# Ellon/pgslam

Hardware: AMD Instinct MI355X
Metric: ICP-converged scans/sec at 100k-pt scan vs 1M-pt local map (higher is better)
Workload: dtype f32; 1 GPU; scan-to-map ICP, 100000-pt Velodyne-shaped scan vs 1000000-pt local map, <=30 iterations (BASELINE.json configs[1]); distinct_scans=64, matcher=grid, streams=1, parallelism=1 independent replica(s), one process per GPU

## Files before the change

pgslam_amd/csrc/k_minimise.inc:

```

__device__ __forceinline__ void accumulate_pair(double *acc, double w, double px, double py, double pz, double qx,
                                                double qy, double qz, double nx, double ny, double nz)
{
    const double dx = px - qx, dy = py - qy, dz = pz - qz;
    const double e = (nx * dx + ny * dy) + nz * dz;
    double J[6];
    J[0] = py * nz - pz * ny;
    J[1] = pz * nx - px * nz;
    J[2] = px * ny - py * nx;
    J[3] = nx; J[4] = ny; J[5] = nz;
    int k = 0;
#pragma unroll
    for (int a = 0; a < 6; a++)
#pragma unroll
        for (int b = a; b < 6; b++) acc[k++] += w * (J[a] * J[b]);
#pragma unroll
    for (int a = 0; a < 6; a++) acc[21 + a] -= w * (J[a] * e);
    acc[27] += w;
    acc[28] += 1.0;
    acc[29] += w * (e * e);
}

template <int NT>
__device__ __forceinline__ void block_reduce_store(double *acc, double *__restrict__ out)
{
    __shared__ double red[kReduceBlock / 64][NT];
    const int lane = threadIdx.x & 63, wid = threadIdx.x >> 6;
#pragma unroll
    for (int k = 0; k < NT; k++) {
        const double v = wave_sum(acc[k]);
        if (lane == 0) red[wid][k] = v;
    }
    __syncthreads();
    if (threadIdx.x < NT) {
        double s = 0.0;
#pragma unroll
        for (int w = 0; w < kReduceBlock / 64; w++) s += red[w][threadIdx.x];
        out[threadIdx.x] = s;
    }
}

template <typename T>
__device__ __forceinline__ void accumulate_pair_p2p(double *acc, double w, T px, T py, T pz, T qx, T qy, T qz)
{
    const double p[3] = {(double)px, (double)py, (double)pz}, q[3] = {(double)qx, (double)qy, (double)qz};
#pragma unroll
    for (int a = 0; a < 3; a++) { acc[a] += w * p[a]; acc[3 + a] += w * q[a]; }
#pragma unroll
    for (int a = 0; a < 3; a++)
#pragma unroll
        for (int b = 0; b < 3; b++) acc[6 + 3 * a + b] += w * (q[a] * p[b]);
    const double dx = (double)(T)(px - qx), dy = (double)(T)(py - qy), dz = (double)(T)(pz - qz);
    acc[27] += w;
    acc[28] += 1.0;
    acc[29] += sqrt((dx * dx + dy * dy) + dz * dz);
}

template <typename T>
__device__ __forceinline__ void normalized3(T &x, T &y, T &z)
{
    const T zz = (x * x + y * y) + z * z;
    if (zz > (T)0) { const T s = sqrt(zz); x = x / s; y = y / s; z = z / s; }
}

template <typename T>
__device__ __forceinline__ T robust_weight(const RobustDev<T> &rb, T dd, T s2)
{
    const T e2 = dd / s2;
    T w = (T)0;
    switch (rb.fct) {
    case 1: w = (T)1 / ((T)1 + e2 / rb.k2); break;
    case 2: w = exp(-(e2 / rb.k2)); break;
    case 3: { const T t = rb.k + e2; w = e2 >= rb.k ? ((T)4 * rb.k2) / (t * t) : (T)1; break; }
    case 4: { const T t = rb.k + e2; w = rb.k2 / (t * t); break; }
    case 5: { const T t = (T)1 - e2 / rb.k2; w = e2 >= rb.k2 ? (T)0 : t * t; break; }
    case 6: w = e2 >= rb.k2 ? rb.k / sqrt_rn_t(e2) : (T)1; break;
    default: w = (T)1 / sqrt_rn_t(e2); break;
    }
    if (sizeof(T) == 8 && w <= (T)1e-50) w = (T)1e-50;
    if (rb.cut && e2 >= rb.a2) w = (T)0;
    return w;
}

template <typename T>
__device__ __forceinline__ T gd_weight(int mode, T thr, T v, T gmax)
{
    if (mode == PGICP_DESC_FILTER_LARGER) return v > thr ? (T)1 : (T)0;
    if (mode == PGICP_DESC_FILTER_SMALLER) return v < thr ? (T)1 : (T)0;
    return gmax > (T)0 ? v / gmax : (T)0;
}

template <typename T, typename S>
__device__ __forceinline__ T pair_filter_weight(const S *Tc, bool use_nrm, const T *qn, T bx, T by, T bz, T normal_cos, bool robust,
                                                const RobustDev<T> &rb, T dd, T rs2, bool gd, int gd_mode, T gd_thr, T gv, T gmax)
{
    if (use_nrm) {
        T ax = ((T)Tc[0] * qn[0] + (T)Tc[1] * qn[1]) + (T)Tc[2] * qn[2];
        T ay = ((T)Tc[4] * qn[0] + (T)Tc[5] * qn[1]) + (T)Tc[6] * qn[2];
        T az = ((T)Tc[8] * qn[0] + (T)Tc[9] * qn[1]) + (T)Tc[10] * qn[2];
        normalized3<T>(ax, ay, az);
        normalized3<T>(bx, by, bz);
        if (((ax * bx + ay * by) + az * bz) < normal_cos) return (T)0;
    }
    T w = (T)1;
    if (robust) w = robust_weight<T>(rb, dd, rs2);
    if (gd) w = w * gd_weight<T>(gd_mode, gd_thr, gv, gmax);
    return w;
}

template <typename T, int MIN, bool GEN>
__global__ __launch_bounds__(kReduceBlock) void k_p2plane_reduce(const ProblemDev *__restrict__ probs,
                                                                  const MapDev<T> *__restrict__ maps,
                                                                  const T *__restrict__ rd_pre, const T *__restrict__ rd_nrm,
                                                                  const int *__restrict__ slot,
                                                                  const T *__restrict__ d2, double *__restrict__ partials,
                                                                  int max_blocks, const int *__restrict__ active, T normal_cos, RobustDev<T> rb,
                                                                  const int *__restrict__ scan_pos, int gd_mode, T gd_thr)
{
    const int prob = active[blockIdx.y];
    const ProblemDev &P = probs[prob];
    if (P.done) return;
    const int tile = xcd_tile(blockIdx.x, gridDim.x);
    const bool robust = GEN && rb.fct != 0;
    const T rs2 = (T)P.robust_s2;
    const int knn = GEN ? P.knn : 1;
    const int np = GEN ? pairs_n(P) : P.n;
    const long long poff = GEN ? pairs_off(P) : P.off;
    if (tile * kReduceSpan >= np) return;
    const MapDev<T> M = maps[P.map];
    const T limit = (T)P.limit;
    const bool use_nrm = GEN && rd_nrm != nullptr;
    const bool need_nrm = MIN == 0 || use_nrm;
    const bool gd = GEN && gd_mode != PGICP_DESC_FILTER_OFF;
    const T gmax = GEN ? Bits<T>::val((typename Bits<T>::U)P.gd_key) : (T)0;
    double acc[kSys];
#pragma unroll
    for (int k = 0; k < kSys; k++) acc[k] = 0.0;
    using V4 = typename Vec4<T>::type;
    for (int rnd = 0; rnd < kReduceRounds; ++rnd) {
    const int base = tile * kReduceSpan + rnd * (kReduceBlock * kReduceItems);
    if (base >= np) break;
    int ss[kReduceItems];
    bool keep[kReduceItems];
    T dds[GEN ? kReduceItems : 1];
    int es[kReduceItems];
#pragma unroll
    for (int it = 0; it < kReduceItems; it++) {
        const int pos = base + it * kReduceBlock + threadIdx.x;
        int e = pos;
        if (scan_pos && pos < np) e = knn == 1 ? scan_pos[P.off + pos] : scan_pos[P.off + pos / knn] * knn + pos % knn;
        es[it] = e;
        ss[it] = -1;
        T dd = Bits<T>::inf();
        if (pos < np) { dd = d2[poff + e]; ss[it] = slot[poff + e]; }
        keep[it] = ss[it] >= 0 && dd <= limit;
        if constexpr (GEN) dds[it] = dd;
    }
    V4 mp[kReduceItems], mn[kReduceItems];
    T qv[kReduceItems][3], qn[kReduceItems][3];
    T gv[GEN ? kReduceItems : 1];
#pragma unroll
    for (int it = 0; it < kReduceItems; it++) {
        const int e = es[it];
        const int s = keep[it] ? ss[it] : 0;
        const int i = keep[it] ? (knn == 1 ? e : e / knn) : 0;
        if (need_nrm) { mp[it] = M.nrm[2 * (long long)s]; mn[it] = M.nrm[2 * (long long)s + 1]; }
        else mp[it] = M.pts[s];
        const T *q = rd_pre + 3 * (P.off + i);
        qv[it][0] = q[0]; qv[it][1] = q[1]; qv[it][2] = q[2];
        if constexpr (GEN) {
            if (use_nrm) { const T *n = rd_nrm + 3 * (P.off + i); qn[it][0] = n[0]; qn[it][1] = n[1]; qn[it][2] = n[2]; }
            if (gd) gv[it] = M.val[s - (keep[it] ? M.first : 0)];
        }
    }
#pragma unroll
    for (int it = 0; it < kReduceItems; it++) {
        if (keep[it]) {
            double wgt = 1.0;
            if constexpr (GEN) {
                const T w = pair_filter_weight<T>(tcur_of<T>(P), use_nrm, qn[it], use_nrm ? mn[it].x : (T)0, use_nrm ? mn[it].y : (T)0,
                                                  use_nrm ? mn[it].z : (T)0, normal_cos, robust, rb, dds[it], rs2, gd, gd_mode, gd_thr,
                                                  gd ? gv[it] : (T)0, gmax);
                if (w == (T)0) continue;
                wgt = (double)w;
            }
            T px, py, pz;
            apply_T<T>(tcur_of<T>(P), qv[it][0], qv[it][1], qv[it][2], px, py, pz);
            if (MIN == 0)
                accumulate_pair(acc, wgt, (double)px, (double)py, (double)pz, (double)mp[it].x, (double)mp[it].y, (double)mp[it].z,
                                (double)mn[it].x, (double)mn[it].y, (double)mn[it].z);
            else
                accumulate_pair_p2p<T>(acc, wgt, px, py, pz, mp[it].x, mp[it].y, mp[it].z);
        }
    }
    }
    block_reduce_store<kSys>(acc, partials + ((long long)prob * max_blocks + tile) * kSys);
}

template <typename T, int MIN>
__global__ __launch_bounds__(kReduceBlock) void k_error_stats(const MapDev<T> *__restrict__ maps, int map,
                                                               const int *__restrict__ slot_of, const T *__restrict__ rd,
                                                               int stride, const int *__restrict__ ids,
                                                               const T *__restrict__ w, int n, int knn, T mx, T my, T mz,
                                                               double *__restrict__ partials)
{
    const MapDev<T> M = maps[map];
    double acc[kSys];
#pragma unroll
    for (int k = 0; k < kSys; k++) acc[k] = 0.0;
    for (int it = 0; it < kReduceItems * kReduceRounds; it++) {
        const int e = blockIdx.x * kReduceSpan + it * kReduceBlock + threadIdx.x;
        if (e < n * knn) {
            const int i = knn == 1 ? e : e / knn;
            const T wi = w[e];
            const int id = ids[e];
            if (id >= 0 && wi != (T)0) {
                const T px = rd[(long long)i * stride] - mx, py = rd[(long long)i * stride + 1] - my,
                        pz = rd[(long long)i * stride + 2] - mz;
                const int s = slot_of[id];
                const auto mp = M.pts[s];
                if (MIN == 0) {
                    const auto mn = M.nrm[2 * (long long)s + 1];
                    accumulate_pair(acc, (double)wi, (double)px, (double)py, (double)pz, (double)mp.x, (double)mp.y,
                                    (double)mp.z, (double)mn.x, (double)mn.y, (double)mn.z);
                } else
                    accumulate_pair_p2p<T>(acc, (double)wi, px, py, pz, mp.x, mp.y, mp.z);
            }
        }
    }
    block_reduce_store<kSys>(acc, partials + (long long)blockIdx.x * kSys);
}

__device__ __forceinline__ double sum_partials_256(const double *__restrict__ part, int nb, int nt, double (*lds)[32])
{
    const int v = threadIdx.x & 31, grp = threadIdx.x >> 5;
    double s = 0.0;
    if (v < nt)
        for (int b = grp; b < nb; b += 8) s += part[(long long)b * nt + v];
    lds[grp][v] = s;
    __syncthreads();
    double tot = 0.0;
    if (threadIdx.x < 32) {
#pragma unroll
        for (int k = 0; k < 8; k++) tot += lds[k][threadIdx.x];
    }
    return tot;
}

__global__ __launch_bounds__(256) void k_sum_partials(const double *__restrict__ partials, int max_blocks, int nt,
                                                       const ProblemDev *__restrict__ probs ,
                                                       int nb_uniform, double *__restrict__ out)
{
    const int p = blockIdx.x;
    int nb = nb_uniform;
    if (probs) {
        nb = (pairs_n(probs[p]) + kReduceSpan - 1) / kReduceSpan;
        if (probs[p].status != PGICP_ST_OK) nb = 0;
    }
    __shared__ double red[8][32];
    const double *src = partials + (long long)p * max_blocks * nt;
    for (int v0 = 0; v0 < nt; v0 += 32) {
        const int v = threadIdx.x & 31, grp = threadIdx.x >> 5;
        double s = 0.0;
        if (v0 + v < nt)
            for (int b = grp; b < nb; b += 8) s += src[(long long)b * nt + v0 + v];
        __syncthreads();
        red[grp][v] = s;
        __syncthreads();
        if (threadIdx.x < 32 && v0 + threadIdx.x < nt) {
            double tot = 0.0;
#pragma unroll
            for (int k = 0; k < 8; k++) tot += red[k][threadIdx.x];
            out[(long long)p * nt + v0 + threadIdx.x] = tot;
        }
    }
}

__device__ __forceinline__ void single_bookkeeping(int *single_host_flag, int *__restrict__ single_stamp,
                                                   int *__restrict__ single_queue_counters, int done)
{
    if (!single_stamp) return;
    const int stamp = *single_stamp + 1;
    *single_stamp = stamp;
    if (single_queue_counters)
        for (int t = 0; t < 4; ++t) { single_queue_counters[8 + t] = single_queue_counters[t]; single_queue_counters[t] = 0; }
    if (single_host_flag) {
        __hip_atomic_store(single_host_flag, done, __ATOMIC_RELAXED, __HIP_MEMORY_SCOPE_SYSTEM);
        __hip_atomic_store(single_host_flag + 1, stamp, __ATOMIC_RELEASE, __HIP_MEMORY_SCOPE_SYSTEM);
    }
}

template <typename T>
__global__ __launch_bounds__(256) void k_solve_update(ProblemDev *__restrict__ probs, const double *__restrict__ partials,
                                                       int max_blocks, ChainDev<T> ch, int *__restrict__ n_done,
                                                       const int *__restrict__ active, int *single_host_flag,
                                                       int *__restrict__ single_stamp, int *__restrict__ single_queue_counters)
{
    const int prob = active[blockIdx.x];
    ProblemDev &P = probs[prob];
    if (P.done) {
        if (threadIdx.x == 0) single_bookkeeping(single_host_flag, single_stamp, single_queue_counters, 1);
        return;
    }
    __shared__ double sys[kSys];
    __shared__ double red[8][32];
    const int nb = (pairs_n(P) + kReduceSpan - 1) / kReduceSpan;
    const double tot = sum_partials_256(partials + (long long)prob * max_blocks * kSys, nb, kSys, red);
    if (threadIdx.x < kSys) {
        sys[threadIdx.x] = tot;
        P.sys[threadIdx.x] = tot;
    }
    __syncthreads();
    if (threadIdx.x != 0) return;
    P.gd_last = P.gd_key;
    P.gd_key = 0;
    int status = PGICP_ST_OK;
    if (P.n_finite == 0 || !(sys[28] > 0.0)) status = PGICP_ST_NO_MATCH;
    if (status == PGICP_ST_OK) {
        double x[6], dT[16], Tn[16];
        if (ch.minimizer == 1) P.rank = solve_p2point(sys, dT);
        else if (ch.force4dof) {
            double s4[27];
            for (int i = 0; i < 27; i++) s4[i] = sys[i];
            constrain_4dof(s4);
            P.rank = solve6(s4, ch.rank_rel_tol, x) - 2;
            delta_T(x, dT);
        }
        else {
            P.rank = solve6(sys, ch.rank_rel_tol, x);
            delta_T(x, dT);
        }
        for (int i = 0; i < 16; i++) { P.T_prev[i] = P.T_iter[i]; P.dT[i] = dT[i]; }
        mat4_mul(dT, P.T_iter, Tn);
        for (int i = 0; i < 16; i++) P.T_iter[i] = Tn[i];
        for (int i = 0; i < 12; i++) { P.Tcur_prev[i] = P.Tcur[i]; P.Tcur[i] = Tn[i]; P.Tcur_prev_f[i] = P.Tcur_f[i]; P.Tcur_f[i] = (float)Tn[i]; }
        P.n_kept = (int)sys[28];
        P.iters += 1;
        const int f = checker_check(P.chk, Tn, ch.max_iters, ch.min_rot, ch.min_trans, ch.smooth, ch.bound_rot, ch.bound_trans);
        if (f & 8) status = PGICP_ST_NAN;
        else if (f & 16) status = PGICP_ST_BOUND;
        else {
            if (f & 2) P.converged = 1;
            if (f & 4) P.max_iter_reached = 1;
            if (!(f & 1)) { P.done = 1; atomicAdd(n_done, 1); }
        }
    }
    if (status != PGICP_ST_OK) {
        P.status = status;
        P.done = 1;
        atomicAdd(n_done, 1);
    }
    single_bookkeeping(single_host_flag, single_stamp, single_queue_counters, P.done ? 1 : 0);
}

__global__ __launch_bounds__(1024) void k_compact_active(const ProblemDev *__restrict__ probs, int P, int *__restrict__ active,
                                                         int *host_flag, int *__restrict__ stamp_counter, int *__restrict__ queue_counters)
{
    int stamp = 0;
    if (threadIdx.x == 0) { stamp = *stamp_counter + 1; *stamp_counter = stamp; }
    if (queue_counters && threadIdx.x < 4) { queue_counters[8 + threadIdx.x] = queue_counters[threadIdx.x]; queue_counters[threadIdx.x] = 0; }
    __shared__ int lds[32];
    __shared__ int base_live, base_done;
    if (threadIdx.x == 0) { base_live = 0; base_done = 0; }
    __syncthreads();
    int live_cnt = 0;
    for (int p = threadIdx.x; p < P; p += 1024) live_cnt += probs[p].done ? 0 : 1;
    int tot;
    block_exclusive_scan_1024(live_cnt, lds, tot);
    const int n_live = tot;
    for (int b = 0; b < P; b += 1024) {
        const int p = b + threadIdx.x;
        const int is_live = (p < P && !probs[p].done) ? 1 : 0;
        const int is_done = (p < P && probs[p].done) ? 1 : 0;
        int tl, td;
        const int el = block_exclusive_scan_1024(is_live, lds, tl);
        const int ed = block_exclusive_scan_1024(is_done, lds, td);
        if (is_live) active[base_live + el] = p;
        if (is_done) active[n_live + base_done + ed] = p;
        __syncthreads();
        if (threadIdx.x == 0) { base_live += tl; base_done += td; }
        __syncthreads();
    }
    if (host_flag && threadIdx.x == 0) {
        __hip_atomic_store(host_flag, P - n_live, __ATOMIC_RELAXED, __HIP_MEMORY_SCOPE_SYSTEM);
        __hip_atomic_store(host_flag + 1, stamp, __ATOMIC_RELEASE, __HIP_MEMORY_SCOPE_SYSTEM);
    }
}

__global__ __launch_bounds__(256) void k_reopen(ProblemDev *__restrict__ probs, int P)
{
    const int p = blockIdx.x * blockDim.x + threadIdx.x;
    if (p < P && probs[p].status == PGICP_ST_OK) probs[p].done = 0;
}
void launch_reopen(hipStream_t st, ProblemDev *probs, int P)
{
    hipLaunchKernelGGL(k_reopen, dim3((P + 255) / 256), dim3(256), 0, st, probs, P);
}

int knn_trace_set(int sorted_index)
{
#ifdef PGICP_KNN_STATS
    return hipMemcpyToSymbol(HIP_SYMBOL(g_trace_i), &sorted_index, sizeof(int)) == hipSuccess ? 0 : -1;
#else
    (void)sorted_index;
    return -1;
#endif
}

int knn_phase_read(unsigned long long out[48], int reset)
{
#ifdef PGICP_PHASE_STATS
    static unsigned long long h[64 * 48];
    if (hipMemcpyFromSymbol(h, HIP_SYMBOL(g_phase), sizeof h) != hipSuccess) return -1;
    for (int k = 0; k < 48; k++) {
        out[k] = 0;
        const bool is_max = k == 32 + 12 || k == 32 + 13;
        for (int c = 0; c < 64; c++) out[k] = is_max ? std::max(out[k], h[c * 48 + k]) : out[k] + h[c * 48 + k];
    }
    if (reset) { std::memset(h, 0, sizeof h); (void)hipMemcpyToSymbol(HIP_SYMBOL(g_phase), h, sizeof h); }
    {
        unsigned long long b[16];
        if (hipMemcpyFromSymbol(b, HIP_SYMBOL(g_ball), sizeof b) == hipSuccess && b[0])
            std::fprintf(stderr, "      ball walk: %llu waves; per wave: %.1f open lanes, %.1f trips, %.1f items in %.2f evaluations; %.1f rows per open lane\n",
                         b[0], (double)b[1] / b[0], (double)b[2] / b[0], (double)b[4] / b[0], (double)b[5] / b[0], b[1] ? (double)b[7] / b[1] : 0.0);
        if (reset) { std::memset(b, 0, sizeof b); (void)hipMemcpyToSymbol(HIP_SYMBOL(g_ball), b, sizeof b); }
    }
    {
        unsigned long long w[16];
        if (hipMemcpyFromSymbol(w, HIP_SYMBOL(g_slow_worst), sizeof w) == hipSuccess && w[0])
            std::fprintf(stderr, "      slowest entry: %llu cycles [fetch %llu seed %llu look-ups %llu points %llu walk %llu finish %llu]; square of %llu rows, %llu with points, %llu long, %llu candidates; bounded %llu capped %llu, result at %llu mm\n",
                         w[0], w[1], w[2], w[3], w[4], w[5], w[6], w[8], w[9], w[10], w[11], w[12], w[13], w[14]);
        if (reset) { std::memset(w, 0, sizeof w); (void)hipMemcpyToSymbol(HIP_SYMBOL(g_slow_worst), w, sizeof w); }
    }
    return 0;
#else
    (void)out; (void)reset;
    return -1;
#endif
}

int knn_stats_read(unsigned long long out[56], int reset)
{
#ifdef PGICP_KNN_STATS
    if (hipMemcpyFromSymbol(out, HIP_SYMBOL(g_knn_stats), 56 * sizeof(unsigned long long)) != hipSuccess) return -1;
    if (reset) { unsigned long long z[56] = {0}; (void)hipMemcpyToSymbol(HIP_SYMBOL(g_knn_stats), z, sizeof z); }
    return 0;
#else
    (void)out; (void)reset;
    return -1;
#endif
}

int knn_dump_setup(long long total, int passes)
{
#ifdef PGICP_KNN_STATS
    unsigned *c = nullptr; float *d = nullptr;
    if (hipMalloc((void **)&c, sizeof(unsigned) * total * passes) != hipSuccess || hipMalloc((void **)&d, sizeof(float) * total * passes) != hipSuccess) return -1;
    (void)hipMemset(c, 0, sizeof(unsigned) * total * passes);
    (void)hipMemset(d, 0, sizeof(float) * total * passes);
    (void)hipMemcpyToSymbol(HIP_SYMBOL(g_cnt_dump), &c, sizeof c);
    (void)hipMemcpyToSymbol(HIP_SYMBOL(g_d2_dump), &d, sizeof d);
    (void)hipMemcpyToSymbol(HIP_SYMBOL(g_dump_total), &total, sizeof total);
    (void)hipMemcpyToSymbol(HIP_SYMBOL(g_dump_passes), &passes, sizeof passes);
    return 0;
#else
    (void)total; (void)passes;
    return -1;
#endif
}
int knn_dump_read(unsigned *cnt, float *d2, long long n)
{
#ifdef PGICP_KNN_STATS
    unsigned *c = nullptr; float *d = nullptr;
    (void)hipDeviceSynchronize();
    (void)hipMemcpyFromSymbol(&c, HIP_SYMBOL(g_cnt_dump), sizeof c);
    (void)hipMemcpyFromSymbol(&d, HIP_SYMBOL(g_d2_dump), sizeof d);
    if (!c || !d) return -1;
    if (hipMemcpy(cnt, c, sizeof(unsigned) * n, hipMemcpyDeviceToHost) != hipSuccess || hipMemcpy(d2, d, sizeof(float) * n, hipMemcpyDeviceToHost) != hipSuccess) return -1;
    return 0;
#else
    (void)cnt; (void)d2; (void)n;
    return -1;
#endif
}

void launch_compact_active(hipStream_t st, const ProblemDev *probs, int P, int *active, int *host_flag, int *stamp_counter,
                           int *queue_counters)
{
    hipLaunchKernelGGL(k_compact_active, dim3(1), dim3(1024), 0, st, probs, P, active, host_flag, stamp_counter, queue_counters);
}

template <typename T, bool GD>
__global__ __launch_bounds__(kReduceBlock) void k_cov_reduce(const ProblemDev *__restrict__ probs,
                                                              const MapDev<T> *__restrict__ maps,
                                                              const T *__restrict__ rd_pre, const T *__restrict__ rd_nrm,
                                                              const int *__restrict__ slot,
                                                              const T *__restrict__ d2, double *__restrict__ partials,
                                                              int max_blocks, T normal_cos, RobustDev<T> rb, const int *__restrict__ scan_pos,
                                                              int gd_mode, T gd_thr)
{
    const ProblemDev &P = probs[blockIdx.y];
    if (P.status != PGICP_ST_OK) return;
    const int np = pairs_n(P), knn = P.knn;
    const long long poff = pairs_off(P);
    if (blockIdx.x * kReduceSpan >= np) return;
    const MapDev<T> M = maps[P.map];
    const T limit = (T)P.limit;
    double alpha, beta, gamma;
    small_angles(P.dT, alpha, beta, gamma);
    const double t_x = P.dT[3], t_y = P.dT[7], t_z = P.dT[11];
    double Tp[12];
#pragma unroll
    for (int k = 0; k < 12; k++) Tp[k] = P.T_prev[k];
    double acc[kCovTerms];
#pragma unroll
    for (int k = 0; k < kCovTerms; k++) acc[k] = 0.0;
    for (int it = 0; it < kReduceItems * kReduceRounds; it++) {
        const int pos = blockIdx.x * kReduceSpan + it * kReduceBlock + threadIdx.x;
        if (pos >= np) continue;
        const int e = !scan_pos ? pos : knn == 1 ? scan_pos[P.off + pos] : scan_pos[P.off + pos / knn] * knn + pos % knn;
        const T dd = d2[poff + e];
        const int s = slot[poff + e];
        if (s < 0 || !(dd <= limit)) continue;
        if constexpr (GD) {
            T w = rb.fct != 0 ? robust_weight<T>(rb, dd, (T)P.robust_s2) : (T)1;
            w = w * gd_weight<T>(gd_mode, gd_thr, M.val[s - M.first], Bits<T>::val((typename Bits<T>::U)P.gd_last));
            if (w == (T)0) continue;
        } else {
            if (rb.fct != 0 && robust_weight<T>(rb, dd, (T)P.robust_s2) == (T)0) continue;
        }
        const int i = knn == 1 ? e : e / knn;
        const T *q = rd_pre + 3 * (P.off + i);
        T pxt, pyt, pzt;
        apply_T<T>(Tp, q[0], q[1], q[2], pxt, pyt, pzt);
        const auto mp = M.nrm[2 * (long long)s];
        const auto mn = M.nrm[2 * (long long)s + 1];
        if (rd_nrm) {
            const T *n = rd_nrm + 3 * (P.off + i);
            T ax = ((T)Tp[0] * n[0] + (T)Tp[1] * n[1]) + (T)Tp[2] * n[2];
            T ay = ((T)Tp[4] * n[0] + (T)Tp[5] * n[1]) + (T)Tp[6] * n[2];
            T az = ((T)Tp[8] * n[0] + (T)Tp[9] * n[1]) + (T)Tp[10] * n[2];
            T bx = mn.x, by = mn.y, bz = mn.z;
            normalized3<T>(ax, ay, az);
            normalized3<T>(bx, by, bz);
            if (((ax * bx + ay * by) + az * bz) < normal_cos) continue;
        }
        const double px = pxt, py = pyt, pz = pzt, qx = mp.x, qy = mp.y, qz = mp.z, nx = mn.x, ny = mn.y, nz = mn.z;
        const double rr = sqrt((px * px + py * py) + pz * pz);
        const double rdx = px / rr, rdy = py / rr, rdz = pz / rr;
        const double qr = sqrt((qx * qx + qy * qy) + qz * qz);
        const double qdx = qx / qr, qdy = qy / qr, qdz = qz / qr;
        const double n_alpha = nz * rdy - ny * rdz;
        const double n_beta = nx * rdz - nz * rdx;
        const double n_gamma = ny * rdx - nx * rdy;
        double E = nx * (px - gamma * py + beta * pz + t_x - qx);
        E += ny * (gamma * px + py - alpha * pz + t_y - qy);
        E += nz * (-beta * px + alpha * py + pz + t_z - qz);
        double Nr = nx * (rdx - gamma * rdy + beta * rdz);
        Nr += ny * (gamma * rdx + rdy - alpha * rdz);
        Nr += nz * (-beta * rdx + alpha * rdy + rdz);
        const double Nq = -((nx * qdx + ny * qdy) + nz * qdz);
        const double er = E + rr * Nr;
        const double h[6] = {nx, ny, nz, rr * n_alpha, rr * n_beta, rr * n_gamma};
        const double gr[6] = {nx * Nr, ny * Nr, nz * Nr, n_alpha * er, n_beta * er, n_gamma * er};
        const double gq[6] = {nx * Nq, ny * Nq, nz * Nq, qr * n_alpha * Nq, qr * n_beta * Nq, qr * n_gamma * Nq};
        int k = 0;
#pragma unroll
        for (int a = 0; a < 6; a++)
#pragma unroll
            for (int b = a; b < 6; b++) {
                acc[k] += h[a] * h[b];
                acc[21 + k] += gr[a] * gr[b] + gq[a] * gq[b];
                k++;
            }
    }
    block_reduce_store<kCovTerms>(acc, partials + ((long long)blockIdx.y * max_blocks + blockIdx.x) * kCovTerms);
}


__global__ __launch_bounds__(64) void k_robust_open(ProblemDev *__restrict__ probs, const int *__restrict__ active, int n_active)
{
    const int a = blockIdx.x * blockDim.x + threadIdx.x;
    if (a >= n_active) return;
    ProblemDev &P = probs[active[a]];
    if (P.done) return;
    P.limit = __longlong_as_double(0x7FF0000000000000LL);
    P.rlimit = P.limit;
}
__global__ __launch_bounds__(64) void k_gd_open(ProblemDev *__restrict__ probs, const int *__restrict__ active, int n_active)
{
    const int a = blockIdx.x * blockDim.x + threadIdx.x;
    if (a >= n_active) return;
    ProblemDev &P = probs[active[a]];
    if (P.done) return;
    P.limit = __longlong_as_double(0x7FF0000000000000LL);
    P.rlimit = P.limit;
    P.n_refined = 1;
}
constexpr int kGdMaxItems = 16;
template <typename T>
__global__ __launch_bounds__(256) void k_gd_max(ProblemDev *__restrict__ probs, const MapDev<T> *__restrict__ maps,
                                                const int *__restrict__ slot, const int *__restrict__ active)
{
    using U = typename Bits<T>::U;
    ProblemDev &P = probs[active[blockIdx.y]];
    if (P.done) return;
    const int np = pairs_n(P);
    const int base = blockIdx.x * (256 * kGdMaxItems);
    if (base >= np) return;
    const MapDev<T> M = maps[P.map];
    const long long poff = pairs_off(P);
    int ss[kGdMaxItems];
#pragma unroll
    for (int it = 0; it < kGdMaxItems; it++) {
        const int e = base + it * 256 + threadIdx.x;
        ss[it] = e < np ? slot[poff + e] : -1;
    }
    U k = 0;
#pragma unroll
    for (int it = 0; it < kGdMaxItems; it++)
        if (ss[it] >= 0) { const T v = M.val[ss[it] - M.first]; if (v > (T)0) k = max(k, Bits<T>::key(v)); }
    __shared__ U red[4];
    for (int o = 32; o > 0; o >>= 1) { const U t = __shfl_xor(k, o); k = t > k ? t : k; }
    if ((threadIdx.x & 63) == 0) red[threadIdx.x >> 6] = k;
    __syncthreads();
    if (threadIdx.x == 0) {
        for (int w = 1; w < 4; w++) k = red[w] > k ? red[w] : k;
        if (k) atomicMax(&P.gd_key, (unsigned long long)k);
    }
}

template <typename T>
__global__ __launch_bounds__(256) void k_robust_absdev(const ProblemDev *__restrict__ probs, const T *__restrict__ d2, T *__restrict__ dev,
                                                       const int *__restrict__ active)
{
    const ProblemDev &P = probs[active[blockIdx.y]];
    if (P.done) return;
    const int e = blockIdx.x * blockDim.x + threadIdx.x;
    if (e >= pairs_n(P)) return;
    const T med = (T)P.qraw, v = d2[pairs_off(P) + e];
    dev[pairs_off(P) + e] = v > med ? v - med : med - v;
}
template <typename T>
__global__ __launch_bounds__(64) void k_robust_finish(ProblemDev *__restrict__ probs, const int *__restrict__ active, int n_active, int mad, T outlier_max_d2)
{
    const int a = blockIdx.x * blockDim.x + threadIdx.x;
    if (a >= n_active) return;
    ProblemDev &P = probs[active[a]];
    if (P.done) return;
    T s2 = (T)1;
    if (mad) { const T sc = sqrt_rn_t((T)P.qraw); s2 = sc * sc; }
    P.robust_s2 = (double)s2;
    P.limit = (double)outlier_max_d2;
    P.rlimit = __longlong_as_double(0x7FF0000000000000LL);
    P.n_refined = 0;
}

template <typename T>
__global__ __launch_bounds__(256) void k_robust_absdev_raw(const T *__restrict__ d2, int n, const T *__restrict__ stat, T *__restrict__ dev)
{
    const int i = blockIdx.x * blockDim.x + threadIdx.x;
    if (i >= n) return;
    const T med = stat[0], v = d2[i];
    dev[i] = v > med ? v - med : med - v;
}
template <typename T>
__global__ __launch_bounds__(256) void k_robust_weights_raw(const T *__restrict__ d2, int n, RobustDev<T> rb, const T *__restrict__ stat,
                                                             T *__restrict__ w)
{
    const int i = blockIdx.x * blockDim.x + threadIdx.x;
    if (i >= n) return;
    T s2 = (T)1;
    if (rb.mad) { const T sc = sqrt_rn_t(stat[2]); s2 = sc * sc; }
    const T v = d2[i];
    w[i] = v == __builtin_huge_val() ? (T)0 : robust_weight<T>(rb, v, s2);
}


template <typename T>
__global__ __launch_bounds__(256) void k_map_values(const typename Vec4<T>::type *__restrict__ pts, int first, int m,
                                                    const T *__restrict__ values, int stride, T *__restrict__ out, int *__restrict__ flags)
{
    const int s = blockIdx.x * blockDim.x + threadIdx.x;
    if (s >= m) return;
    const T v = values[(long long)Bits<T>::unpack_idx(pts[first + s].w) * stride];
    out[s] = v;
    if (!isfinite(v)) atomicOr(flags, 1);
    else if (v < (T)0) atomicOr(flags + 1, 1);
}
```

pgslam_amd/csrc/kernels.hip:

```cpp
#include "kernels.hpp"
#include <algorithm>
#include <cstdio>
#include <cstdlib>
#include <cstring>
#include <limits>
#include <map>
#include <type_traits>
#ifndef PGICP_FAST_BLOCK
#define PGICP_FAST_BLOCK 64
#endif
#ifndef PGICP_FAST_WAVES
#define PGICP_FAST_WAVES 6
#endif
#ifndef PGICP_FAST_ATTR
#ifndef PGICP_FAST_WAVES_D
#define PGICP_FAST_WAVES_D 4
#endif
#define PGICP_FAST_ATTR __attribute__((amdgpu_num_sgpr(80), amdgpu_waves_per_eu(sizeof(T) == 4 ? PGICP_FAST_WAVES : PGICP_FAST_WAVES_D, sizeof(T) == 4 ? PGICP_FAST_WAVES : PGICP_FAST_WAVES_D)))
#endif

namespace pgicp {

template <typename T> struct Bits;
template <> struct Bits<float> {
    using U = unsigned int;
    static constexpr int kBits = 32;
    __device__ static U key(float v) { return __float_as_uint(v); }
    __device__ static float val(U k) { return __uint_as_float(k); }
    __device__ static float pack_idx(int i) { return __int_as_float(i); }
    __device__ static int unpack_idx(float w) { return __float_as_int(w); }
    __device__ static float inf() { return __uint_as_float(0x7F800000u); }
};
template <> struct Bits<double> {
    using U = unsigned long long;
    static constexpr int kBits = 64;
    __device__ static U key(double v) { return (U)__double_as_longlong(v); }
    __device__ static double val(U k) { return __longlong_as_double((long long)k); }
    __device__ static double pack_idx(int i) { return __longlong_as_double((long long)i); }
    __device__ static int unpack_idx(double w) { return (int)__double_as_longlong(w); }
    __device__ static double inf() { return __longlong_as_double(0x7FF0000000000000LL); }
};

__device__ __forceinline__ float4 make_v4(float x, float y, float z, float w) { return make_float4(x, y, z, w); }
__device__ __forceinline__ double4 make_v4(double x, double y, double z, double w) { return make_double4(x, y, z, w); }

__device__ __forceinline__ int xcd_tile(int b, int nb)
{
    const int q = nb >> 3, r = nb & 7;
    const int xcd = b & 7, j = b >> 3;
    return xcd * q + (xcd < r ? xcd : r) + j;
}

__device__ __forceinline__ double wave_sum(double v)
{
#pragma unroll
    for (int o = 32; o > 0; o >>= 1) v += __shfl_down(v, o, 64);
    return v;
}

template <typename T, typename S>
__device__ __forceinline__ void apply_T(const S *Tc, T x, T y, T z, T &ox, T &oy, T &oz)
{
    const T r00 = (T)Tc[0], r01 = (T)Tc[1], r02 = (T)Tc[2], tx = (T)Tc[3];
    const T r10 = (T)Tc[4], r11 = (T)Tc[5], r12 = (T)Tc[6], ty = (T)Tc[7];
    const T r20 = (T)Tc[8], r21 = (T)Tc[9], r22 = (T)Tc[10], tz = (T)Tc[11];
    ox = ((r00 * x + r01 * y) + r02 * z) + tx;
    oy = ((r10 * x + r11 * y) + r12 * z) + ty;
    oz = ((r20 * x + r21 * y) + r22 * z) + tz;
}

template <typename T> __device__ __forceinline__ auto tcur_of(const ProblemDev &P)
{
    if constexpr (sizeof(T) == 4) return (const float *)P.Tcur_f; else return (const double *)P.Tcur;
}
template <typename T> __device__ __forceinline__ auto tcur_prev_of(const ProblemDev &P)
{
    if constexpr (sizeof(T) == 4) return (const float *)P.Tcur_prev_f; else return (const double *)P.Tcur_prev;
}

template <typename V>
__device__ __forceinline__ const __attribute__((address_space(1))) V *as_global(const V *p)
{
    return (const __attribute__((address_space(1))) V *)p;
}
template <typename T> struct Raw4;
template <> struct Raw4<float> { typedef float type __attribute__((ext_vector_type(4))); };
template <> struct Raw4<double> { typedef double type __attribute__((ext_vector_type(4))); };
template <typename T, int K = 0>
__device__ __forceinline__ typename Vec4<T>::type load_rec(const typename Vec4<T>::type *p, int j)
{
    using R4 = typename Raw4<T>::type;
    const R4 r = as_global(reinterpret_cast<const R4 *>(p))[j + K];
    return make_v4(r.x, r.y, r.z, r.w);
}
__device__ __forceinline__ int load_tab(const int *p, int i)
{
    return as_global(p)[i];
}

__device__ __forceinline__ int succ_rank(const uint4 w, int k)
{
    const unsigned long long m = ((unsigned long long)w.y << 32) | w.x;
    return (int)w.z + __popcll(m & ((1ULL << k) - 1ULL));
}
__device__ __forceinline__ uint4 load_word(const uint4 *sw, int g)
{
    typedef unsigned U4 __attribute__((ext_vector_type(4)));
    const U4 r = as_global(reinterpret_cast<const U4 *>(sw))[g];
    return make_uint4(r.x, r.y, r.z, r.w);
}
template <bool SUCC, typename T>
__device__ __forceinline__ int tab_fine(const MapDev<T> &M, int f)
{
    if constexpr (SUCC) return load_tab(M.ostart, succ_rank(load_word(M.sw, f >> 6), f & 63));
    else return load_tab(M.cell_start_f, f);
}
template <bool SUCC, typename T>
__device__ __forceinline__ void tab_range(const MapDev<T> &M, int ia, int ib, int &a, int &b)
{
    if constexpr (SUCC) {
        const uint4 wa = load_word(M.sw, ia >> 6), wb = load_word(M.sw, ib >> 6);
        const int ra = succ_rank(wa, ia & 63), rb = succ_rank(wb, ib & 63);
        a = 0; b = 0;
        if (ra != rb) { a = load_tab(M.ostart, ra); b = load_tab(M.ostart, rb); }
    } else { a = load_tab(M.cell_start_f, ia); b = load_tab(M.cell_start_f, ib); }
}
template <typename T> __device__ __forceinline__ int tab_fine_any(const MapDev<T> &M, int f) { return M.sw ? tab_fine<true, T>(M, f) : tab_fine<false, T>(M, f); }
template <typename T> __device__ __forceinline__ void tab_range_any(const MapDev<T> &M, int ia, int ib, int &a, int &b)
{
    if (M.sw) tab_range<true, T>(M, ia, ib, a, b); else tab_range<false, T>(M, ia, ib, a, b);
}
template <int TK, typename T> __device__ __forceinline__ void tab_range_k(const MapDev<T> &M, int ia, int ib, int &a, int &b)
{
    if constexpr (TK == 2) tab_range_any<T>(M, ia, ib, a, b); else tab_range<TK == 1, T>(M, ia, ib, a, b);
}
template <typename T> __device__ __forceinline__ int tab_coarse_any(const MapDev<T> &M, int c) { return M.sw ? tab_fine<true, T>(M, c * M.kx) : load_tab(M.cell_start, c); }

__device__ __forceinline__ int pairs_n(const ProblemDev &P) { return P.n * P.knn; }
__device__ __forceinline__ long long pairs_off(const ProblemDev &P) { return P.off * P.knn; }

#include "k_build.inc"
#include "k_sort.inc"
#include "k_mapbuild.inc"
#include "k_match.inc"
#include "k_normals.inc"
#include "k_select.inc"
#include "k_minimise.inc"
#include "k_filter.inc"
#include "k_axisquantile.inc"
#include "k_launch.inc"
#include "k_ssn.inc"
#include "k_vartrim.inc"
#include "k_pairsort.inc"
#include "k_voxel.inc"
#include "k_noise.inc"
#include "k_density.inc"
#include "k_covsample.inc"
#include "k_octree.inc"
#include "k_normalspace.inc"

}
```

Baseline: 11490 scans/s.

## Fold block reductions across lanes with DPP/permlane and batch covariance gathers

Replaces the per-term wave_sum loop in block_reduce_store with a transpose-style fold that uses permlane32/16 swaps and DPP row operations. Each level halves the number of live values while combining lane halves, so each lane ends up owning one of the NT sums, which it then writes to shared memory. The covariance kernel is restructured to batch kReduceItems gathers (d2, slot, map records, scan points, normals, gd values) before computing, to raise memory-level parallelism. Map record loads also go through explicit global address-space vector loads. This adds code complexity, depends on gfx950-specific permlane swap intrinsics, and increases register pressure from the batched arrays.

```diff
diff --git a/pgslam_amd/csrc/k_minimise.inc b/pgslam_amd/csrc/k_minimise.inc
--- a/pgslam_amd/csrc/k_minimise.inc
+++ b/pgslam_amd/csrc/k_minimise.inc
@@ -21,16 +21,91 @@
     acc[29] += w * (e * e);
 }
 
+constexpr int kDppShl4 = 0x104, kDppShr4 = 0x114, kDppRor8 = 0x128, kDppQuadXor2 = 0x4E, kDppQuadXor1 = 0xB1;
+
+__host__ __device__ constexpr int fold_lane(int k)
+{
+    return ((k & 1) << 5) | ((k & 2) << 3) | ((k & 4) << 1) | ((k & 8) >> 1) | ((k & 16) >> 3) | ((k & 32) >> 5);
+}
+
+__device__ __forceinline__ double fold_pack(unsigned lo, unsigned hi) { return __hiloint2double((int)hi, (int)lo); }
+__device__ __forceinline__ unsigned fold_lo(double v) { return (unsigned)__double2loint(v); }
+__device__ __forceinline__ unsigned fold_hi(double v) { return (unsigned)__double2hiint(v); }
+
+template <int O>
+__device__ __forceinline__ double fold_swap_add(double a, double b)
+{
+    static_assert(O == 32 || O == 16, "swap levels");
+    unsigned al = fold_lo(a), ah = fold_hi(a), bl = fold_lo(b), bh = fold_hi(b);
+    if constexpr (O == 32) {
+        const auto l = __builtin_amdgcn_permlane32_swap(al, bl, false, false);
+        const auto h = __builtin_amdgcn_permlane32_swap(ah, bh, false, false);
+        al = l[0]; bl = l[1]; ah = h[0]; bh = h[1];
+    } else {
+        const auto l = __builtin_amdgcn_permlane16_swap(al, bl, false, false);
+        const auto h = __builtin_amdgcn_permlane16_swap(ah, bh, false, false);
+        al = l[0]; bl = l[1]; ah = h[0]; bh = h[1];
+    }
+    return fold_pack(al, ah) + fold_pack(bl, bh);
+}
+
+template <int CTRL, int BANKS>
+__device__ __forceinline__ double fold_dpp(double keep, double src)
+{
+    const unsigned lo = (unsigned)__builtin_amdgcn_update_dpp((int)fold_lo(keep), (int)fold_lo(src), CTRL, 0xF, BANKS, false);
+    const unsigned hi = (unsigned)__builtin_amdgcn_update_dpp((int)fold_hi(keep), (int)fold_hi(src), CTRL, 0xF, BANKS, false);
+    return fold_pack(lo, hi);
+}
+
+template <int O>
+__device__ __forceinline__ double fold_row_add(double a, double b, int lane)
+{
+    if constexpr (O == 8)
+        return fold_dpp<kDppRor8, 0xC>(a, b) + fold_dpp<kDppRor8, 0x3>(b, a);
+    else if constexpr (O == 4)
+        return fold_dpp<kDppShr4, 0xA>(a, b) + fold_dpp<kDppShl4, 0x5>(b, a);
+    else {
+        const bool up = (lane & O) != 0;
+        const double own = up ? b : a, sent = up ? a : b;
+        return own + fold_dpp<O == 2 ? kDppQuadXor2 : kDppQuadXor1, 0xF>(sent, sent);
+    }
+}
+
+template <int O>
+__device__ __forceinline__ double fold_pair(double a, double b, int lane)
+{
+    if constexpr (O >= 16) return fold_swap_add<O>(a, b); else return fold_row_add<O>(a, b, lane);
+}
+
+template <int O, int N>
+__device__ __forceinline__ void fold_level(double *v, int lane)
+{
+#pragma unroll
+    for (int j = 0; j < (N + 1) / 2; j++) v[j] = fold_pair<O>(v[2 * j], 2 * j + 1 < N ? v[2 * j + 1] : v[2 * j], lane);
+}
+
+template <int NT>
+__device__ __forceinline__ double wave_fold(double *v, int lane)
+{
+    static_assert(NT >= 1 && NT <= 64, "one lane per sum");
+    constexpr int n1 = (NT + 1) / 2, n2 = (n1 + 1) / 2, n3 = (n2 + 1) / 2, n4 = (n3 + 1) / 2, n5 = (n4 + 1) / 2;
+    fold_level<32, NT>(v, lane);
+    fold_level<16, n1>(v, lane);
+    fold_level<8, n2>(v, lane);
+    fold_level<4, n3>(v, lane);
+    fold_level<2, n4>(v, lane);
+    fold_level<1, n5>(v, lane);
+    return v[0];
+}
+
 template <int NT>
 __device__ __forceinline__ void block_reduce_store(double *acc, double *__restrict__ out)
 {
     __shared__ double red[kReduceBlock / 64][NT];
     const int lane = threadIdx.x & 63, wid = threadIdx.x >> 6;
-#pragma unroll
-    for (int k = 0; k < NT; k++) {
-        const double v = wave_sum(acc[k]);
-        if (lane == 0) red[wid][k] = v;
-    }
+    const double v = wave_fold<NT>(acc, lane);
+    const int k = fold_lane(lane);
+    if (k < NT) red[wid][k] = v;
     __syncthreads();
     if (threadIdx.x < NT) {
         double s = 0.0;
@@ -164,13 +239,13 @@
         const int e = es[it];
         const int s = keep[it] ? ss[it] : 0;
         const int i = keep[it] ? (knn == 1 ? e : e / knn) : 0;
-        if (need_nrm) { mp[it] = M.nrm[2 * (long long)s]; mn[it] = M.nrm[2 * (long long)s + 1]; }
-        else mp[it] = M.pts[s];
+        if (need_nrm) { mp[it] = map_rec<T>(M.nrm, 2 * (long long)s); mn[it] = map_rec<T>(M.nrm, 2 * (long long)s + 1); }
+        else mp[it] = map_rec<T>(M.pts, s);
         const T *q = rd_pre + 3 * (P.off + i);
         qv[it][0] = q[0]; qv[it][1] = q[1]; qv[it][2] = q[2];
         if constexpr (GEN) {
             if (use_nrm) { const T *n = rd_nrm + 3 * (P.off + i); qn[it][0] = n[0]; qn[it][1] = n[1]; qn[it][2] = n[2]; }
-            if (gd) gv[it] = M.val[s - (keep[it] ? M.first : 0)];
+            if (gd) gv[it] = as_global(M.val)[s - (keep[it] ? M.first : 0)];
         }
     }
 #pragma unroll
@@ -218,9 +293,9 @@
                 const T px = rd[(long long)i * stride] - mx, py = rd[(long long)i * stride + 1] - my,
                         pz = rd[(long long)i * stride + 2] - mz;
                 const int s = slot_of[id];
-                const auto mp = M.pts[s];
+                const auto mp = map_rec<T>(M.pts, s);
                 if (MIN == 0) {
-                    const auto mn = M.nrm[2 * (long long)s + 1];
+                    const auto mn = map_rec<T>(M.nrm, 2 * (long long)s + 1);
                     accumulate_pair(acc, (double)wi, (double)px, (double)py, (double)pz, (double)mp.x, (double)mp.y,
                                     (double)mp.z, (double)mn.x, (double)mn.y, (double)mn.z);
                 } else
@@ -515,28 +590,57 @@
     double acc[kCovTerms];
 #pragma unroll
     for (int k = 0; k < kCovTerms; k++) acc[k] = 0.0;
-    for (int it = 0; it < kReduceItems * kReduceRounds; it++) {
-        const int pos = blockIdx.x * kReduceSpan + it * kReduceBlock + threadIdx.x;
-        if (pos >= np) continue;
-        const int e = !scan_pos ? pos : knn == 1 ? scan_pos[P.off + pos] : scan_pos[P.off + pos / knn] * knn + pos % knn;
-        const T dd = d2[poff + e];
-        const int s = slot[poff + e];
-        if (s < 0 || !(dd <= limit)) continue;
+    using V4 = typename Vec4<T>::type;
+    const bool use_nrm = rd_nrm != nullptr;
+    for (int rnd = 0; rnd < kReduceRounds; ++rnd) {
+    const int base = blockIdx.x * kReduceSpan + rnd * (kReduceBlock * kReduceItems);
+    if (base >= np) break;
+    int ss[kReduceItems], es[kReduceItems];
+    bool keep[kReduceItems];
+    T dds[kReduceItems];
+#pragma unroll
+    for (int it = 0; it < kReduceItems; it++) {
+        const int pos = base + it * kReduceBlock + threadIdx.x;
+        int e = pos;
+        if (scan_pos && pos < np) e = knn == 1 ? scan_pos[P.off + pos] : scan_pos[P.off + pos / knn] * knn + pos % knn;
+        es[it] = e;
+        ss[it] = -1;
+        T dd = Bits<T>::inf();
+        if (pos < np) { dd = d2[poff + e]; ss[it] = slot[poff + e]; }
+        keep[it] = ss[it] >= 0 && dd <= limit;
+        dds[it] = dd;
+    }
+    V4 mps[kReduceItems], mns[kReduceItems];
+    T qv[kReduceItems][3], qn[kReduceItems][3];
+    T gv[GD ? kReduceItems : 1];
+#pragma unroll
+    for (int it = 0; it < kReduceItems; it++) {
+        const int e = es[it];
+        const int s = keep[it] ? ss[it] : 0;
+        const int i = keep[it] ? (knn == 1 ? e : e / knn) : 0;
+        mps[it] = map_rec<T>(M.nrm, 2 * (long long)s);
+        mns[it] = map_rec<T>(M.nrm, 2 * (long long)s + 1);
+        const T *q = rd_pre + 3 * (P.off + i);
+        qv[it][0] = q[0]; qv[it][1] = q[1]; qv[it][2] = q[2];
+        if (use_nrm) { const T *n = rd_nrm + 3 * (P.off + i); qn[it][0] = n[0]; qn[it][1] = n[1]; qn[it][2] = n[2]; }
+        if constexpr (GD) gv[it] = as_global(M.val)[s - (keep[it] ? M.first : 0)];
+    }
+#pragma unroll
+    for (int it = 0; it < kReduceItems; it++) {
+        if (!keep[it]) continue;
+        const T dd = dds[it];
         if constexpr (GD) {
             T w = rb.fct != 0 ? robust_weight<T>(rb, dd, (T)P.robust_s2) : (T)1;
-            w = w * gd_weight<T>(gd_mode, gd_thr, M.val[s - M.first], Bits<T>::val((typename Bits<T>::U)P.gd_last));
+            w = w * gd_weight<T>(gd_mode, gd_thr, gv[it], Bits<T>::val((typename Bits<T>::U)P.gd_last));
             if (w == (T)0) continue;
         } else {
             if (rb.fct != 0 && robust_weight<T>(rb, dd, (T)P.robust_s2) == (T)0) continue;
         }
-        const int i = knn == 1 ? e : e / knn;
-        const T *q = rd_pre + 3 * (P.off + i);
         T pxt, pyt, pzt;
-        apply_T<T>(Tp, q[0], q[1], q[2], pxt, pyt, pzt);
-        const auto mp = M.nrm[2 * (long long)s];
-        const auto mn = M.nrm[2 * (long long)s + 1];
-        if (rd_nrm) {
-            const T *n = rd_nrm + 3 * (P.off + i);
+        apply_T<T>(Tp, qv[it][0], qv[it][1], qv[it][2], pxt, pyt, pzt);
+        const V4 mp = mps[it], mn = mns[it];
+        if (use_nrm) {
+            const T *n = qn[it];
             T ax = ((T)Tp[0] * n[0] + (T)Tp[1] * n[1]) + (T)Tp[2] * n[2];
             T ay = ((T)Tp[4] * n[0] + (T)Tp[5] * n[1]) + (T)Tp[6] * n[2];
             T az = ((T)Tp[8] * n[0] + (T)Tp[9] * n[1]) + (T)Tp[10] * n[2];
@@ -574,6 +678,7 @@
                 k++;
             }
     }
+    }
     block_reduce_store<kCovTerms>(acc, partials + ((long long)blockIdx.y * max_blocks + blockIdx.x) * kCovTerms);
 }
 
diff --git a/pgslam_amd/csrc/kernels.hip b/pgslam_amd/csrc/kernels.hip
--- a/pgslam_amd/csrc/kernels.hip
+++ b/pgslam_amd/csrc/kernels.hip
@@ -93,6 +93,13 @@
     const R4 r = as_global(reinterpret_cast<const R4 *>(p))[j + K];
     return make_v4(r.x, r.y, r.z, r.w);
 }
+template <typename T>
+__device__ __forceinline__ typename Vec4<T>::type map_rec(const typename Vec4<T>::type *p, long long j)
+{
+    using R4 = typename Raw4<T>::type;
+    const R4 r = as_global(reinterpret_cast<const R4 *>(p))[j];
+    return make_v4(r.x, r.y, r.z, r.w);
+}
 __device__ __forceinline__ int load_tab(const int *p, int i)
 {
     return as_global(p)[i];
```

New measurement: 11880 scans/s, median of 6. 1.03x the previous value.
